# kcroker/Gadget-2.0.7-ngravs

Hardware: AMD Instinct MI355X
Metric: particle-steps/s (tree+PM) (higher is better)
Workload: dtype f64

## Files before the change

### gadget-2.0.7-ngravs_amd/__init__.py

```python
import ctypes as C
import os
import subprocess

import numpy as np

from . import abi, ic
from .abi import (Config, Particles, Stats, make_config, WALK_GROUP, WALK_STRICT,
                  LAW_NONE, LAW_NEWTON, LAW_NEG_NEWTON, LAW_YUKAWA, LAW_COLOYUK, LAW_BAMBAM, LAW_SOURCEBAM, LAW_TARGETBAM)

_HERE = os.path.dirname(os.path.abspath(__file__))
LIB_PATH = os.path.join(_HERE, "libngravs_hip.so")
_LIB = None

EXPORTS = [
    "ngravs_abi_version", "ngravs_build_info", "ngravs_config_default", "ngravs_create", "ngravs_create_with_laws", "ngravs_destroy",
    "ngravs_last_walk_kernel", "ngravs_shortrange_table_with_laws", "ngravs_user_table_eval",
    "ngravs_set_fatal_handler", "ngravs_set_opening", "ngravs_set_walk_mode", "ngravs_set_softening", "ngravs_dd_record_bytes", "ngravs_get_config", "ngravs_set_tuning",
    "ngravs_memcpy", "ngravs_device_alloc", "ngravs_device_free",
    "ngravs_set_particles",
    "ngravs_set_old_acc", "ngravs_update_particles", "ngravs_force_update_tree", "ngravs_domain_decomposition", "ngravs_discard_grav_pm",
    "ngravs_force_treebuild", "ngravs_gravity_tree",
    "ngravs_pmforce_periodic", "ngravs_compute_accelerations", "ngravs_get_accel", "ngravs_get_stats", "ngravs_walk_unopened",
    "ngravs_get_domain", "ngravs_get_keys", "ngravs_get_order", "ngravs_get_shard", "ngravs_last_error",
    "ngravs_peano_hilbert_key", "ngravs_peano_keys", "ngravs_shortrange_table", "ngravs_direct_sum", "ngravs_direct_sum_targets",
    "ngravs_dd_num_local", "ngravs_dd_local_extent", "ngravs_dd_set_extent", "ngravs_get_domain_extent", "ngravs_dd_set_toptree",
    "ngravs_dd_get_toptree", "ngravs_dd_peano_order", "ngravs_dd_leaf_sums", "ngravs_dd_target_bounds", "ngravs_dd_keep_margin", "ngravs_dd_pack", "ngravs_dd_get_dest",
    "ngravs_dd_pack_leaves", "ngravs_dd_set_top", "ngravs_dd_recv_buffer", "ngravs_dd_apply_migration", "ngravs_dd_set_halo",
    "ngravs_dd_leaf_sums_kept", "ngravs_dd_pack_leaves_kept", "ngravs_dd_refresh_halo", "ngravs_dd_update_top", "ngravs_dd_get_kept",
    "ngravs_dd_set_ids", "ngravs_dd_get_ids",
    "ngravs_pm_slab_begin", "ngravs_pm_slab_pack", "ngravs_pm_slab_unpack", "ngravs_pm_slab_bytes",
]
HOST_EXPORTS = ["ngravs_host_comm_selftest", "ngravs_host_kept_step", "ngravs_host_toptree_borrow", "ngravs_host_domain_decomposition", "ngravs_host_domain_owners", "ngravs_host_domain_halo",
                "ngravs_host_plan_free", "ngravs_host_pmforce_periodic", "ngravs_host_compute_accelerations", "ngravs_host_split",
                "ngravs_host_pm_seconds", "ngravs_host_toptree_init", "ngravs_host_toptree_from_children", "ngravs_host_toptree_adapt",
                "ngravs_host_toptree_free", "ngravs_host_import_request", "ngravs_host_import_request_margin"]
RCCL_LIB_PATH = os.path.join(_HERE, "libngravs_rccl.so")
RCCL_EXPORTS = ["ngravs_rccl_selftest", "ngravs_rccl_unique_id", "ngravs_rccl_create", "ngravs_rccl_fill", "ngravs_rccl_destroy", "ngravs_rccl_stats",
                "ngravs_rccl_last_error", "ngravs_rccl_world", "ngravs_rccl_barrier", "ngravs_rccl_set_timeout"]

# ... 43 lines not shown
        L.ngravs_get_keys.argtypes = [C.c_void_p, C.c_void_p, C.c_int]
        L.ngravs_get_order.argtypes = [C.c_void_p, C.c_void_p, C.c_int]
        L.ngravs_get_shard.argtypes = [C.c_void_p, C.c_void_p, C.c_void_p]
        L.ngravs_peano_keys.argtypes = [C.c_void_p, C.c_void_p, C.c_int64, C.c_void_p, C.c_double, C.c_int, C.c_void_p]
        L.ngravs_shortrange_table.argtypes = [C.c_void_p, C.c_void_p, C.c_void_p]
        L.ngravs_direct_sum.argtypes = [C.c_void_p, C.c_void_p, C.c_int64, C.c_void_p]
        L.ngravs_direct_sum_targets.argtypes = [C.c_void_p, C.c_void_p, C.c_void_p, C.c_void_p, C.c_int64, C.c_void_p]
        L.ngravs_dd_local_extent.argtypes = [C.c_void_p, C.c_void_p, C.c_void_p]
        L.ngravs_dd_set_extent.argtypes = [C.c_void_p, C.c_void_p, C.c_void_p]
        L.ngravs_get_config.argtypes = [C.c_void_p, C.c_void_p]
        L.ngravs_host_split.argtypes = [C.c_void_p, C.c_void_p, C.c_int64, C.c_int, C.c_double, C.c_void_p]
        L.ngravs_dd_pack.argtypes = [C.c_void_p, C.c_int, C.c_void_p, C.c_int, C.c_int, C.c_void_p, C.c_void_p, C.c_void_p]
        L.ngravs_host_toptree_init.argtypes = [C.c_void_p, C.c_int]
        L.ngravs_host_toptree_from_children.argtypes = [C.c_void_p, C.c_void_p, C.c_int32]
        L.ngravs_host_toptree_adapt.argtypes = [C.c_void_p, C.c_void_p, C.c_double, C.c_int, C.c_void_p]
        L.ngravs_host_toptree_free.argtypes = [C.c_void_p]
        L.ngravs_host_toptree_free.restype = None
        L.ngravs_host_import_request.argtypes = [C.c_void_p, C.c_void_p, C.c_void_p, C.c_void_p, C.c_void_p, C.c_int, C.c_void_p, C.c_void_p]
        L.ngravs_dd_apply_migration.argtypes = [C.c_void_p, C.c_void_p, C.c_int64]
        L.ngravs_dd_set_halo.argtypes = [C.c_void_p, C.c_void_p, C.c_int64]
        L.ngravs_dd_set_ids.argtypes = [C.c_void_p, C.c_void_p, C.c_int]
        L.ngravs_create_with_laws.argtypes = [C.c_void_p, C.c_void_p, C.c_int, C.c_void_p]
        L.ngravs_last_walk_kernel.argtypes = [C.c_void_p]
        L.ngravs_shortrange_table_with_laws.argtypes = [C.c_void_p, C.c_void_p, C.c_int, C.c_void_p, C.c_void_p]
        L.ngravs_user_table_eval.argtypes = [C.c_void_p, C.c_double, C.c_double, C.c_double, C.c_void_p, C.c_int64, C.c_void_p,
                                             C.c_void_p]
        L.ngravs_dd_get_ids.argtypes = [C.c_void_p, C.c_void_p, C.c_int]
        _LIB = L
    return _LIB


def shard_range(n, rank, world_size):
    lo = (n * rank) // world_size
    hi = (n * (rank + 1)) // world_size
    lo = (lo // 64) * 64
    hi = n if rank + 1 == world_size else (hi // 64) * 64
    return lo, hi - lo


def peano_hilbert_key(x, y, z, bits):
    return int(lib().ngravs_peano_hilbert_key(int(x), int(y), int(z), int(bits)))


def shortrange_table(cfg):
    ng = cfg.n_gravs
    force = np.zeros((ng, ng, abi.NTAB))
# ... 28 lines not shown
    return out, err.value


def _ptr(a):
    return a.ctypes.data if a is not None else None


class Engine:

    def __init__(self, cfg, user_fns=None):
        self.cfg = cfg
        self._h = C.c_void_p()
        self._user_arr, nfns, self._user_keep = abi.user_registry(user_fns)
        rc = lib().ngravs_create_with_laws(C.byref(cfg), self._user_arr, nfns, C.byref(self._h))
        if rc != 0:
            msg = lib().ngravs_last_error(None)
            self.status = rc
            raise NgravsError("ngravs_create failed with status %d (no HIP device or bad wiring): %s" % (rc, msg.decode() if msg else ""))
        self._keep = []
        self.n = 0

    def last_walk_kernel(self):
        return int(lib().ngravs_last_walk_kernel(self._h))

    def close(self):
        if self._h:
            lib().ngravs_destroy(self._h)
            self._h = C.c_void_p()

    def __del__(self):
        try:
            self.close()
        except Exception:
            pass

    def _check(self, rc, what):
        if rc != 0:
            msg = lib().ngravs_last_error(self._h)
            raise NgravsError("%s failed: status %d (%s)" % (what, rc, msg.decode() if msg else ""))

    def _host_columns(self, pos, mass, ptype, old_acc, active, grav_pm, grav_cost=None):
        pos = np.ascontiguousarray(pos, dtype=np.float64)
        mass = np.ascontiguousarray(mass, dtype=np.float64)
        ptype = np.ascontiguousarray(ptype, dtype=np.int32)
        p = Particles()
        p.n = len(pos)
# ... 176 lines not shown
```

### gadget-2.0.7-ngravs_amd/csrc/capi.hip

```cpp
#include "engine.hpp"
#include "../../include/ngravs_peano.h"
#include <chrono>
#include <cmath>

static thread_local std::string g_create_error;

void ngravs_report(ngravs_ctx *ctx, int code, const std::string &msg)
{
  if(ctx)
    ctx->last_error = msg;
  else
    g_create_error = msg;
  if(ctx && ctx->on_fatal)
    ctx->on_fatal(code, msg.c_str());
  else
    fprintf(stderr, "task %d: endrun called with an error level of %d (%s)\n", ctx ? ctx->cfg.rank : 0, code, msg.c_str());
}

__global__ void k_pack_strided_f64(const unsigned char *src, long long stride, int ncomp, long long n, double *dst)
{
  long long i = blockIdx.x * (long long)blockDim.x + threadIdx.x;
  if(i >= n)
    return;
  const double *s = reinterpret_cast<const double *>(src + i * stride);
// ... 234 lines not shown
  std::string why;
  int rc = check_config(cfg, why);
  if(rc == NGRAVS_OK)
    rc = user_check_config(cfg, fns, nfns, why);
  if(rc != NGRAVS_OK)
    {
      ngravs_report(nullptr, rc, why);
      return rc;
    }
  int ndev = 0;
  if(hipGetDeviceCount(&ndev) != hipSuccess || ndev <= 0)
    {
      ngravs_report(nullptr, NGRAVS_ERR_NO_DEVICE, "no HIP device: libngravs_hip has no CPU fallback");
      return NGRAVS_ERR_NO_DEVICE;
    }
  if(cfg->device < 0 || cfg->device >= ndev)
    return NGRAVS_ERR_ARG;
  ngravs_ctx *c = new ngravs_ctx;
  c->cfg = *cfg;
  c->user_fns.assign(fns, fns + nfns);
  memset(&c->stats, 0, sizeof(c->stats));
  if(hipSetDevice(cfg->device) != hipSuccess || hipStreamCreate(&c->stream) != hipSuccess ||
     hipEventCreate(&c->ev0) != hipSuccess || hipEventCreate(&c->ev1) != hipSuccess ||
     hipEventCreate(&c->evk0) != hipSuccess || hipEventCreate(&c->evk1) != hipSuccess)
    {
      delete c;
      return NGRAVS_ERR_NO_DEVICE;
    }
  if(cfg->pmgrid)
    {
      c->asmth = cfg_asmth(cfg);
      c->rcut = cfg_rcut(cfg);
    }
  *out = c;
  return NGRAVS_OK;
}

extern "C" void ngravs_destroy(ngravs_ctx *c)
{
  if(!c)
    return;
  (void)hipSetDevice(c->cfg.device);
  (void)hipStreamSynchronize(c->stream);
  pm_release(c);
  pmslab_release(c);
  c->in_cost.release();
  c->in_pos.release();
// ... 46 lines not shown
  c->lat.release();
  c->walk_stack.release();
  c->walk_counters.release();
  c->walk_ovf.release();
  c->walk_tlist.release();
  c->walk_tmp.release();
  c->lvl_table.release();
  c->r_acc.release();
  c->r_pm.release();
  c->r_oldacc.release();
  c->r_nint.release();
  c->pm_rho.release();
  c->pm_phi.release();
  c->pm_force.release();
  c->pm_orig.release();
  c->out_tmp.release();
  c->out_tmpf.release();
  (void)hipEventDestroy(c->ev0);
  (void)hipEventDestroy(c->ev1);
  (void)hipEventDestroy(c->evk0);
  (void)hipEventDestroy(c->evk1);
  for(hipEvent_t e : c->ev_batch)
    (void)hipEventDestroy(e);
  (void)hipStreamDestroy(c->stream);
  delete c;
}

extern "C" void ngravs_set_fatal_handler(ngravs_ctx *ctx, ngravs_fatal_fn fn)
{
  if(ctx)
    ctx->on_fatal = fn;
}

extern "C" int ngravs_set_opening(ngravs_ctx *c, double theta, double errtol)
{
  if(!c)
    return NGRAVS_ERR_ARG;
  c->cfg.err_tol_theta = theta;
  c->cfg.err_tol_force_acc = errtol;
  return NGRAVS_OK;
}

extern "C" int ngravs_set_softening(ngravs_ctx *c, const double force_softening[NGRAVS_NTYPES])
{
  if(!c || !force_softening)
    return NGRAVS_ERR_ARG;
// ... 49 lines not shown
    }
  else if(k == "walk_root")
    t.walk_root = iv != 0;
  else if(k == "walk_compact")
    t.walk_compact = iv != 0;
  else if(k == "walk_spread" && iv >= 0 && iv <= 64 && (iv & (iv - 1)) == 0)
    t.walk_spread = (int)iv;
  else if(k == "walk_sg" && iv >= 0 && iv <= 16)
    t.walk_sg = (int)iv;
  else if(k == "walk_ring" && iv >= 0 && iv <= 1)
    t.walk_ring = (int)iv;
  else if(k == "walk_ring_k" && iv >= 0 && iv <= 8)
    t.walk_ring_k = (int)iv;
  else if(k == "walk_nleaf" && iv >= -1 && iv <= 8)
    t.walk_nleaf = (int)iv;
  else if(k == "walk_exact_reach")
    t.walk_exact_reach = iv != 0;
  else if(k == "sort_full")
    t.sort_full = iv != 0;
  else if(k == "tree_levelwise")
    t.tree_levelwise = iv != 0;
  else if(k == "dd_keep" && v >= 0 && v <= 0.25)
    t.dd_keep = v;
  else
    {
      ngravs_report(c, NGRAVS_ERR_ARG, "ngravs_set_tuning: unknown name or value out of range: " + k);
      return NGRAVS_ERR_ARG;
    }
  return NGRAVS_OK;
}

extern "C" int ngravs_memcpy(ngravs_ctx *c, void *dst, const void *src, int64_t bytes, int kind)
{
  if(!c || bytes < 0 || kind < 1 || kind > 3 || (bytes > 0 && (!dst || !src)))
    return NGRAVS_ERR_ARG;
  if(bytes == 0)
    return NGRAVS_OK;
  (void)hipSetDevice(c->cfg.device);
  HIP_TRY(c, hipStreamSynchronize(c->stream));
  HIP_TRY(c, hipMemcpy(dst, src, (size_t)bytes, kind == 1 ? hipMemcpyHostToDevice : (kind == 2 ? hipMemcpyDeviceToHost : hipMemcpyDeviceToDevice)));
  return NGRAVS_OK;
}

extern "C" int ngravs_device_alloc(ngravs_ctx *c, void **ptr, int64_t bytes)
{
  if(!c || !ptr || bytes < 0)
// ... 42 lines not shown
}

static double ev_ms(ngravs_ctx *c);

static int set_particles_impl(ngravs_ctx *c, const ngravs_particles_t *p, bool keep_tree)
{
  if(!c || !p || p->n < 0 || (p->n > 0 && (!p->pos || !p->mass || !p->type)))
    return NGRAVS_ERR_ARG;
  if(p->n == 0 && keep_tree)
    {
      if(!c->have_particles || c->n_local != 0)
        return NGRAVS_ERR_STATE;
      c->tree_stale = c->have_tree;
      return NGRAVS_OK;
    }
  if(p->n == 0)
    {
      (void)hipSetDevice(c->cfg.device);
      c->n = c->n_local = 0;
      c->own_order_nlocal = -1;
      c->sort_low = 35;
      c->all_active = true;
      c->walk_ia_ratio = 0;
      c->walk_unit_state = 4;
      c->have_particles = true;
      c->have_order = c->have_tree = c->have_pm = c->have_acc = false;
      c->top.on = false;
      c->pm_parked = false;
      return NGRAVS_OK;
    }
  const bool keep_halo = keep_tree && c->n_local != c->n;
  if(keep_tree && (!c->have_order || !c->have_tree || p->n != c->n_local))
    {
      ngravs_report(c, NGRAVS_ERR_STATE, "ngravs_update_particles: needs a built tree over the same own particles");
      return NGRAVS_ERR_STATE;
    }
  if(p->n >= (1ll << 31) - 64)
    {
      ngravs_report(c, NGRAVS_ERR_ARG, "int particle indices (reference All.MaxPart is int): n must be < 2^31");
      return NGRAVS_ERR_ARG;
    }
  (void)hipSetDevice(c->cfg.device);
  const int64_t n = p->n;
  if(c->in_pos.ensure(3 * n) || c->in_mass.ensure(n) || c->in_oldacc.ensure(n) || c->in_type.ensure(n) || c->in_active.ensure(n) ||
     (!keep_tree && c->in_cost.ensure(n)))
    {
// ... 75 lines not shown
        }
      HIP_TRY(c, hipMemcpyAsync(c->in_type.p, h, sizeof(int) * n, hipMemcpyHostToDevice, c->stream));
      HIP_TRY(c, hipStreamSynchronize(c->stream));
    }
  c->all_active = p->active == nullptr;
  if(p->active)
    {
      if(p->on_device)
        hipLaunchKernelGGL(k_pack_active, GRID1(n), 0, c->stream, (const unsigned char *)p->active,
                           (long long)p->active_stride, (long long)n, c->in_active.p);
      else
        {
          c->host_stage.resize((size_t)n);
          for(int64_t i = 0; i < n; i++)
            c->host_stage[i] = ((const unsigned char *)p->active)[i * p->active_stride] ? 1 : 0;
          HIP_TRY(c, hipMemcpyAsync(c->in_active.p, c->host_stage.data(), (size_t)n, hipMemcpyHostToDevice, c->stream));
          HIP_TRY(c, hipStreamSynchronize(c->stream));
        }
    }
  else
    hipLaunchKernelGGL(k_fill_u8, GRID1(n), 0, c->stream, c->in_active.p, (long long)n, (unsigned char)1);
  HIP_TRY(c, hipGetLastError());
  c->walk_ia_ratio = 0;
  c->walk_unit_state = 4;
  c->have_particles = true;
  if(keep_tree)
    c->tree_stale = true;
  else
    {
      c->have_order = c->have_tree = c->have_pm = c->have_acc = false;
      c->top.on = false;
      c->pm_parked = false;
      if(p->grav_pm && c->cfg.pmgrid)
        {
          if(c->pm_orig.ensure(3 * n))
            return NGRAVS_ERR_NOMEM;
          if((rc = upload_column_f64(c, p->grav_pm, p->grav_pm_stride, 3, n, p->on_device, c->pm_orig.p)))
            return rc;
          c->pm_parked = true;
        }
    }
  return NGRAVS_OK;
}

extern "C" int ngravs_set_particles(ngravs_ctx *c, const ngravs_particles_t *p) { return set_particles_impl(c, p, false); }

// ... 156 lines not shown
}

static int ensure_table(ngravs_ctx *c)
{
  if(!c->cfg.pmgrid || c->table_ready)
    return NGRAVS_OK;
  const int ng = c->cfg.n_gravs;
  std::vector<double> h((size_t)(ng * ng + 1) * NTAB);
  host_shortrange_table(&c->cfg, h.data(), nullptr, c->user_fns.data(), (int)c->user_fns.size());
  {
    WalkParams wp;
    make_walk_params(c, &wp);
    for(int t = 0; t < NTAB; t++)
      h[(size_t)ng * ng * NTAB + t] = exp(-wp.ym * (double)t * wp.inv_asmthfac);
  }
  if(c->table.ensure(h.size()))
    return NGRAVS_ERR_NOMEM;
  HIP_TRY(c, hipMemcpyAsync(c->table.p, h.data(), sizeof(double) * h.size(), hipMemcpyHostToDevice, c->stream));
  HIP_TRY(c, hipStreamSynchronize(c->stream));
  c->table_ready = true;
  return NGRAVS_OK;
}

extern "C" int ngravs_gravity_tree(ngravs_ctx *c)
{
  if(!c || !c->have_order)
    return NGRAVS_ERR_STATE;
  (void)hipSetDevice(c->cfg.device);
  int rc;
  if(!c->have_tree)
    {
      int64_t nn = ngravs_force_treebuild(c);
      if(nn < 0)
        return (int)nn;
    }
  else if(c->tree_stale && (rc = ngravs_force_update_tree(c)))
    return rc;
  if((rc = ensure_table(c)))
    return rc;
  if(c->n_local == 0)
    {
      c->stats.t_treewalk = 0;
      c->stats.walk_kernel_ms = 0;
      c->stats.interactions = 0;
      c->stats.n_active = 0;
      c->have_acc = true;
      return NGRAVS_OK;
    }
  HIP_TRY(c, hipEventRecord(c->ev0, c->stream));
  if((rc = walk_run(c)))
    return rc;
  if((rc = walk_finish(c)))
    return rc;
  HIP_TRY(c, hipEventRecord(c->ev1, c->stream));
  c->stats.t_treewalk = ev_ms(c) * 1e-3;
  float kms = 0;
  (void)hipEventSynchronize(c->evk1);
  (void)hipEventElapsedTime(&kms, c->evk0, c->evk1);
  c->stats.walk_kernel_ms = kms;
  double h[2] = {0, 0};
  HIP_TRY(c, hipMemcpyAsync(h, c->red_tmp.p, 2 * sizeof(double), hipMemcpyDeviceToHost, c->stream));
  HIP_TRY(c, hipStreamSynchronize(c->stream));
  c->stats.interactions = h[0];
  c->stats.n_active = (int64_t)h[1];
  c->have_acc = true;
  if(c->cfg.pmgrid && c->cfg.walk_mode == NGRAVS_WALK_GROUP && h[1] > 0 && c->cfg.box_size > 0)
    {
      const double reach = (c->cfg.group_reach > 0 ? c->cfg.group_reach : NGRAVS_GROUP_REACH) * c->asmth;
      const double ntot = c->top.on && c->top.total_count > 0 ? c->top.total_count : (double)c->n;
      const double L = c->cfg.box_size, expect = 4.18879020478639 * reach * reach * reach * ntot / (L * L * L);
      const bool dense = c->walk_ntargets < 0 || c->walk_dense_tlist;
      if(expect > 0 && dense)
        {
          const double f_sg = c->walk_sg >= 4 ? 1.0 : (c->walk_sg >= 2 ? 1857.0 / 1393.0 : 1857.0 / 1079.0);
          const double f_s = c->walk_spread >= 2 ? 1079.0 / 871.0 : 1.0;
          c->walk_ia_ratio = (h[0] / h[1]) / expect * f_sg * f_s;
        }
    }
  if(c->shard_count > 0 && c->extent_override)
    hipLaunchKernelGGL(k_cost_update, GRID1(c->shard_count), 0, c->stream, c->s_idx.p, c->s_active.p, c->r_nint.p,
                       (long long)c->shard_first, (long long)c->shard_count, c->in_cost.p);
  return NGRAVS_OK;
}

extern "C" int ngravs_pmforce_periodic(ngravs_ctx *c)
{
  if(!c || !c->have_particles)
    return NGRAVS_ERR_STATE;
  (void)hipSetDevice(c->cfg.device);
  int rc;
  if(!c->have_order && (rc = ngravs_domain_decomposition(c)))
    return rc;
  if(!c->have_tree)
    {
      int64_t nn = ngravs_force_treebuild(c);
      if(nn < 0)
        return (int)nn;
    }
  else if(c->tree_stale && (rc = ngravs_force_update_tree(c)))
    return rc;
  HIP_TRY(c, hipEventRecord(c->ev0, c->stream));
  if((rc = pm_run(c)))
    return rc;
  HIP_TRY(c, hipEventRecord(c->ev1, c->stream));
  c->stats.t_pm = ev_ms(c) * 1e-3;
  return NGRAVS_OK;
}

extern "C" int ngravs_compute_accelerations(ngravs_ctx *c, int pm_step)
{
  if(!c || !c->have_particles)
    return NGRAVS_ERR_STATE;
  int rc;
  if((rc = domain_decomposition_impl(c, !(pm_step && c->cfg.pmgrid))))
    return rc;
  if(pm_step && c->cfg.pmgrid && (rc = ngravs_pmforce_periodic(c)))
    return rc;
  return ngravs_gravity_tree(c);
}

static int download_strided(ngravs_ctx *c, const void *dsrc, size_t elem, int ncomp, int64_t n, void *dst, int64_t stride,
                            int on_device)
{
  const size_t row = elem * ncomp;
  if(on_device)
    {
      if((size_t)stride != row)
        {
          ngravs_report(c, NGRAVS_ERR_ARG, "device outputs must be contiguous");
          return NGRAVS_ERR_ARG;
        }
      HIP_TRY(c, hipMemcpyAsync(dst, dsrc, row * n, hipMemcpyDeviceToDevice, c->stream));
      HIP_TRY(c, hipStreamSynchronize(c->stream));
      return NGRAVS_OK;
    }
  if((size_t)stride == row)
    {
      HIP_TRY(c, hipMemcpyAsync(dst, dsrc, row * n, hipMemcpyDeviceToHost, c->stream));
      HIP_TRY(c, hipStreamSynchronize(c->stream));
      return NGRAVS_OK;
    }
// ... 196 lines not shown
}

extern "C" int ngravs_get_order(ngravs_ctx *c, int32_t *order, int on_device)
{
  if(!c || !c->have_order || !order)
    return NGRAVS_ERR_STATE;
  (void)hipSetDevice(c->cfg.device);
  return download_strided(c, c->s_idx.p, sizeof(int), 1, c->n, order, sizeof(int), on_device);
}

extern "C" int ngravs_get_shard(ngravs_ctx *c, int64_t *first, int64_t *count)
{
  if(!c || !c->have_order)
    return NGRAVS_ERR_STATE;
  if(first)
    *first = c->shard_first;
  if(count)
    *count = c->shard_count;
  return NGRAVS_OK;
}

extern "C" const char *ngravs_last_error(ngravs_ctx *c) { return c ? c->last_error.c_str() : g_create_error.c_str(); }
extern "C" int ngravs_last_walk_kernel(ngravs_ctx *c) { return c ? c->last_walk_kernel : NGRAVS_ERR_ARG; }

extern "C" int64_t ngravs_peano_hilbert_key(int x, int y, int z, int bits) { return ngravs_ph_key(x, y, z, bits); }

extern "C" int ngravs_peano_keys(ngravs_ctx *c, const double *pos, int64_t n, const double corner[3], double fac, int bits,
                                 int64_t *keys)
{
  if(!c || !pos || !keys || n <= 0 || bits < 1 || bits > 21)
    return NGRAVS_ERR_ARG;
  (void)hipSetDevice(c->cfg.device);
  DevBuf<double> dpos;
  DevBuf<long long> dkeys;
  if(dpos.ensure(3 * n) || dkeys.ensure(n))
    return NGRAVS_ERR_NOMEM;
  int rc = NGRAVS_OK;
  if(hipMemcpyAsync(dpos.p, pos, sizeof(double) * 3 * n, hipMemcpyHostToDevice, c->stream) != hipSuccess)
    rc = NGRAVS_ERR_NO_DEVICE;
  if(!rc)
    rc = dom_keys_only(c, dpos.p, n, corner, fac, bits, dkeys.p);
  if(!rc && hipMemcpyAsync(keys, dkeys.p, sizeof(long long) * n, hipMemcpyDeviceToHost, c->stream) != hipSuccess)
    rc = NGRAVS_ERR_NO_DEVICE;
  (void)hipStreamSynchronize(c->stream);
  dpos.release();
  dkeys.release();
// ... 339 lines not shown
```

### gadget-2.0.7-ngravs_amd/csrc/engine.hpp

```cpp
#pragma once
#include <hip/hip_runtime.h>
#include <cstdint>
#include <cstdio>
#include <cstdlib>
#include <cstring>
#include <string>
#include <vector>
#include "../../include/ngravs_host.h"

#define NG_MAX NGRAVS_MAX_GRAVS
#define NTAB NGRAVS_NTAB
#define TREE_BITS NGRAVS_TREE_BITS
#define FLAG_BUCKET 64
#define FLAG_PSEUDO 128
#define FLAG_PARTIAL 256
#define MAX_LEVELS (TREE_BITS + 1)

struct ngravs_ctx;

#define HIP_TRY(ctx, expr)                                                                        \
  do                                                                                              \
    {                                                                                             \
      hipError_t e__ = (expr);                                                                    \
      if(e__ != hipSuccess)                                                                       \
// ... 106 lines not shown
  UserTabs ut;
};

struct TreeView
{
  const int *first, *count, *child, *flags;
  const int *npart;
  const double4 *geo, *mom;
  int nnodes;
  const int *ltab;
  int ltab_level;
  double ltab_corner[3], ltab_cl;
};

struct Tuning
{
  int walk_fused = 0, walk_waves = 0, walk_lcap = 0, walk_root = 0, walk_compact = 1, walk_spread = 0, walk_exact_reach = 0, walk_sg = 0, walk_nleaf = -1;
  long long walk_batch = 0;
  int sort_full = 0;
  int tree_levelwise = 0;
  double dd_keep = 0;
  int walk_ring = 1;
  int walk_ring_k = 0;
};

#define TOP_CW(ng) (7 + 4 * (ng))
struct TopTree
{
  double total_count = 0;
  bool on = false;
  double import_reach = 0;
  ngravs_toptree h = {0, 0, 0, 0, nullptr, nullptr, nullptr, nullptr, nullptr};
  DevBuf<int> child, leaf;
  DevBuf<int> gcnt;
  DevBuf<unsigned char> info;
  DevBuf<double> gsum;
  DevBuf<int> leaf_owner;
  DevBuf<unsigned long long> reqmask;
  DevBuf<double> leaf_sums;
  DevBuf<int> own_leaf;
  long long own_leaf_n = -1;
  int kept_rank = -1, kept_world = 0;
  std::vector<int> h_leaf_owner;
  std::vector<unsigned char> h_present;
  std::vector<double> h_node_sums;
  DevBuf<int> kept_row;
// ... 98 lines not shown
  DevBuf<int> r_nint;
  int pm_plan_n = 0;
  void *fft_fwd = nullptr, *fft_inv = nullptr;
  DevBuf<double> pm_rho;
  DevBuf<double> pm_force;
  DevBuf<double> pm_phi;
  DevBuf<double> pm_orig;
  DevBuf<double> out_tmp;
  DevBuf<float> out_tmpf;
  std::vector<unsigned char> host_stage;
  ngravs_stats_t stats;
  hipEvent_t ev0 = nullptr, ev1 = nullptr, evk0 = nullptr, evk1 = nullptr;
  std::vector<hipEvent_t> ev_batch;
  int walk_batches = 0;
  int walk_lcap = 0;
  int walk_scap = 0;
  std::string last_error;
  std::vector<ngravs_user_fn_t> user_fns;
  DevBuf<double> user_tab;
  UserTabs user_ut = {};
  bool user_ready = false;
  double user_soft[NGRAVS_NTYPES] = {0, 0, 0, 0, 0, 0};
  int last_walk_kernel = 0;
  DevBuf<double> user_green;
  long long user_green_nk2 = 0;
};

int dom_find_extent(ngravs_ctx *c);
int dom_keys_and_sort(ngravs_ctx *c);
int dom_keys_only(ngravs_ctx *c, const double *d_pos, int64_t n, const double corner[3], double fac, int bits,
                  long long *d_keys);
int dd_local_extent(ngravs_ctx *c, double lo[3], double hi[3]);
void dd_apply_extent(ngravs_ctx *c, const double lo[3], const double hi[3]);
int dd_set_toptree(ngravs_ctx *c, int nnode, const int *child);
int dd_leaf_sums(ngravs_ctx *c, void **dev_sums, int64_t *count);
int dd_pack(ngravs_ctx *c, int what, const int *leaf_owner, int nranks, int me, int64_t *counts, void **dev_records, int64_t *nrec);
int dd_apply_migration(ngravs_ctx *c, const void *dev_records, int64_t nrec);
int dd_get_dest(ngravs_ctx *c, const int *leaf_owner, int *dest);
int dd_target_bounds(ngravs_ctx *c, double out[2]);
int dd_pack_leaves(ngravs_ctx *c, const unsigned long long *reqmask, int nranks, int me, int64_t *counts, void **dev_records, int64_t *nrec);
int dd_set_top(ngravs_ctx *c, const double *node_sums, const unsigned char *present);
int dd_set_halo(ngravs_ctx *c, const void *dev_records, int64_t nrec);
int dd_leaf_sums_kept(ngravs_ctx *c, void **dev_sums, int64_t *count);
int dd_pack_leaves_kept(ngravs_ctx *c, int64_t *counts, void **dev_records, int64_t *nrec);
int dd_refresh_halo(ngravs_ctx *c, const void *dev_records, int64_t nrec);
int dd_update_top(ngravs_ctx *c, const double *node_sums, const double *leaf_len);
int dd_peano_order_own(ngravs_ctx *c, int force);
int dd_fill_ids(ngravs_ctx *c);
// ... 48 lines not shown
```

### gadget-2.0.7-ngravs_amd/csrc/kernels_pm.hip

```cpp
#include "engine.hpp"
#include "pm_common.hpp"
#include <hipfft/hipfft.h>

__global__ void k_cic_deposit(const double4 *__restrict__ s_pm, const unsigned char *__restrict__ s_type,
                              const unsigned char *__restrict__ s_flag, long long n,
                              double to_slab, int N, int ng, const int *__restrict__ t2g_tab, double *__restrict__ rho)
{
  long long i = blockIdx.x * (long long)blockDim.x + threadIdx.x;
  if(i >= n || (s_flag[i] & 2))
    return;
  double4 p = s_pm[i];
  int g = t2g_tab[s_type[i]];
  const long long NZ = N + 2;
  double *grid = rho + (size_t)g * N * N * NZ;
  double dx, dy, dz;
  int sx = cell_of(p.x, to_slab, N, &dx), sy = cell_of(p.y, to_slab, N, &dy), sz = cell_of(p.z, to_slab, N, &dz);
  int sxx = sx + 1 == N ? 0 : sx + 1, syy = sy + 1 == N ? 0 : sy + 1, szz = sz + 1 == N ? 0 : sz + 1;
  double m = p.w;
  atomicAdd(&grid[((long long)sx * N + sy) * NZ + sz], m * (1.0 - dx) * (1.0 - dy) * (1.0 - dz));
  atomicAdd(&grid[((long long)sx * N + syy) * NZ + sz], m * (1.0 - dx) * dy * (1.0 - dz));
  atomicAdd(&grid[((long long)sx * N + sy) * NZ + szz], m * (1.0 - dx) * (1.0 - dy) * dz);
  atomicAdd(&grid[((long long)sx * N + syy) * NZ + szz], m * (1.0 - dx) * dy * dz);
  atomicAdd(&grid[((long long)sxx * N + sy) * NZ + sz], m * (dx) * (1.0 - dy) * (1.0 - dz));
  atomicAdd(&grid[((long long)sxx * N + syy) * NZ + sz], m * (dx)*dy * (1.0 - dz));
// ... 344 lines not shown
  HIP_TRY(c, hipGetLastError());
  return NGRAVS_OK;
}

int pm_deposit(ngravs_ctx *c)
{
  const int N = c->cfg.pmgrid, ng = c->cfg.n_gravs;
  const long long n = c->n;
  if(N <= 0 || !c->cfg.periodic)
    {
      ngravs_report(c, NGRAVS_ERR_ARG, "pmforce_periodic needs PERIODIC and PMGRID");
      return NGRAVS_ERR_ARG;
    }
  const size_t real_elems = (size_t)N * N * (N + 2);
  if(c->pm_rho.ensure(real_elems * ng) || c->pm_phi.ensure(real_elems * ng) || c->r_pm.ensure(3 * n) || c->d_counters.ensure(16))
    return NGRAVS_ERR_NOMEM;
  if(c->pm_plan_n != N)
    {
      pm_release(c);
      c->fft_fwd = new hipfftHandle;
      c->fft_inv = new hipfftHandle;
      FFT_TRY(c, hipfftPlan3d((hipfftHandle *)c->fft_fwd, N, N, N, HIPFFT_D2Z));
      FFT_TRY(c, hipfftPlan3d((hipfftHandle *)c->fft_inv, N, N, N, HIPFFT_Z2D));
      FFT_TRY(c, hipfftSetStream(*(hipfftHandle *)c->fft_fwd, c->stream));
      FFT_TRY(c, hipfftSetStream(*(hipfftHandle *)c->fft_inv, c->stream));
      c->pm_plan_n = N;
    }
  HIP_TRY(c, hipMemcpyAsync(c->d_counters.p + 8, c->cfg.type_to_grav, sizeof(int) * 6, hipMemcpyHostToDevice, c->stream));
  const double L = c->cfg.box_size, to_slab = N / L;
  HIP_TRY(c, hipMemsetAsync(c->pm_rho.p, 0, sizeof(double) * real_elems * ng, c->stream));
  const int bs = 256;
  unsigned nbp = (unsigned)((n + bs - 1) / bs);
  MeshAddr ma;
  ma.N = N;
  ma.brick = 0;
  for(int j = 0; j < 3; j++)
    {
      ma.lo[j] = 0;
      ma.ext[j] = N;
    }
  int rct = pm_deposit_tiles(c, ma, c->pm_rho.p);
  if(rct == 1)
    hipLaunchKernelGGL(k_cic_deposit, dim3(nbp), dim3(bs), 0, c->stream, c->s_pm.p, c->s_type.p, c->s_active.p, n, to_slab, N, ng,
                       c->d_counters.p + 8, c->pm_rho.p);
  else if(rct)
    return rct;
  HIP_TRY(c, hipGetLastError());
  return NGRAVS_OK;
}

// ... 82 lines not shown
```

### gadget-2.0.7-ngravs_amd/csrc/kernels_walk.hip

```cpp
#include "engine.hpp"
#include "walk_device.hpp"
#include "eval_asm.inc"
#include <hipcub/hipcub.hpp>
#include <type_traits>

__device__ __forceinline__ double bam_eta(int law, double target, double m, double N, double eps)
{
  if(law == NGRAVS_LAW_BAMBAM)
    return 4.0 * M_PI * eps / (target + m / N);
  if(law == NGRAVS_LAW_SOURCEBAM)
    return 4.0 * M_PI * eps * N / m;
  return 4.0 * M_PI * eps / target;
}
__device__ __forceinline__ double bam_accel(int law, double target, double m, double r, double N, double eps)
{
  double eta = bam_eta(law, target, m, N, eps), rho = 2 * target * m / M_PI;
  double reta = r * eta, reta2 = reta * reta, eta3 = eta * eta * eta;
  if(reta < 0.1)
    return rho * eta3 * (2.0 * r / 3.0 - 4.0 * reta2 * r / 5.0 + 6.0 * reta2 * reta2 * r / 7.0);
  return rho * eta3 * (atan(reta) / (reta2 * eta) - 1.0 / (reta * eta * (1 + reta2)));
}
__device__ __forceinline__ double bam_spline(int law, double target, double m, double r, double N, double eps)
{
  double eta = bam_eta(law, target, m, N, eps), rho = 2 * target * m / M_PI;
// ... 2103 lines not shown
  c->walk_dense_tlist = false;
  const bool imports = c->n_local != c->n;
  if((c->all_active && !imports) || c->shard_count <= 0 || !c->tune.walk_compact)
    return NGRAVS_OK;
  const int n = (int)c->shard_count;
  if(c->walk_tlist.ensure((size_t)n) || c->walk_counters.ensure(32))
    return NGRAVS_ERR_NOMEM;
  hipcub::CountingInputIterator<int> idx((int)c->shard_first);
  hipcub::TransformInputIterator<bool, ActiveFlag, const unsigned char *> flags(c->s_active.p + c->shard_first, ActiveFlag());
  size_t bytes = 0;
  HIP_TRY(c, hipcub::DeviceSelect::Flagged(nullptr, bytes, idx, flags, c->walk_tlist.p, c->walk_counters.p + 24, n, c->stream));
  if(c->walk_tmp.ensure(bytes))
    return NGRAVS_ERR_NOMEM;
  HIP_TRY(c, hipcub::DeviceSelect::Flagged(c->walk_tmp.p, bytes, idx, flags, c->walk_tlist.p, c->walk_counters.p + 24, n, c->stream));
  int cnt = 0;
  HIP_TRY(c, hipMemcpyAsync(&cnt, c->walk_counters.p + 24, sizeof(int), hipMemcpyDeviceToHost, c->stream));
  HIP_TRY(c, hipStreamSynchronize(c->stream));
  if(4ll * cnt < 3ll * n || imports)
    c->walk_ntargets = cnt;
  c->walk_dense_tlist = imports && 4ll * cnt >= 3ll * c->n_local;
  return NGRAVS_OK;
}

template <int NG, bool PM, bool YUK, bool TAB_LDS, bool LATT, bool USR = false>
static int launch_group2_t(ngravs_ctx *c, const WalkParams &wp, int *glist = nullptr, int nlist = 0)
{
  const int S0 = c->walk_spread > 1 ? c->walk_spread : 1, G0 = (WAVE / S0) * (glist ? c->walk_sg : 1);
  int S = S0;
  if(glist)
    {
      const int want = nlist <= 4096 ? 64 : (nlist <= 65536 ? 8 : 1);
      S = want > S0 ? want : S0;
    }
  const int G = WAVE / S;
  int ncu = 256;
  hipDeviceProp_t prop;
  if(hipGetDeviceProperties(&prop, c->cfg.device) == hipSuccess && prop.multiProcessorCount > 0)
    ncu = prop.multiProcessorCount;
  const size_t fixed = ((PM && TAB_LDS) ? sizeof(double) * (wp.ntab_lds + wp.exp_tab) * NTAB : 0) + 40 * sizeof(double);
  int waves = (int)((160 * 1024 - fixed) / GW2_WAVE_LDS);
  int per_cu = 1;
  if(waves > GW_MAXWAVES)
    waves = GW_MAXWAVES;
  if(waves < 1)
    waves = 1;
  size_t lds = fixed + (size_t)waves * GW2_WAVE_LDS;
  long long ngroups = glist ? (long long)nlist * (G0 / G) : (walk_tcount(c) + G - 1) / G;
  long long nblk = (long long)ncu * per_cu;
  if(nblk > (ngroups + waves - 1) / waves)
    nblk = (ngroups + waves - 1) / waves;
  if(nblk < 1)
    nblk = 1;
  if(c->walk_stack.ensure((size_t)nblk * waves * (GW_STACK + (size_t)NG * GW2_ITEMS)) || c->walk_counters.ensure(32))
    return NGRAVS_ERR_NOMEM;
  if(glist)
    HIP_TRY(c, hipMemsetAsync(c->walk_counters.p + 8, 0, sizeof(int) * 8, c->stream));
  else
    HIP_TRY(c, hipMemsetAsync(c->walk_counters.p, 0, sizeof(int) * 32, c->stream));
  auto kern = k_walk_group2<NG, PM, YUK, TAB_LDS, LATT, 0, USR>;
  HIP_TRY(c, hipFuncSetAttribute(reinterpret_cast<const void *>(kern), hipFuncAttributeMaxDynamicSharedMemorySize, (int)lds));
  hipLaunchKernelGGL(kern, dim3((unsigned)nblk), dim3(waves * 64), lds, c->stream, tree_view(c), c->s_pm.p,
                     c->s_type.p, c->s_oldacc.p, c->s_active.p, LATT ? c->lat.p : c->table.p, wp, (long long)c->shard_first,
                     walk_tcount(c), c->walk_counters.p, c->walk_stack.p, c->walk_counters.p + 1, c->r_acc.p,
                     c->r_nint.p, (int *)nullptr, (int *)nullptr, 0ll, glist ? (long long)nlist : 0ll, 0, 0, glist, S, G0, walk_tlist(c), 1);
  return NGRAVS_OK;
}

template <int NG, bool PM, bool YUK, bool TAB_LDS, bool LATT, bool USR = false> static int launch_group3_t(ngravs_ctx *c, const WalkParams &wp)
{
  int ncu = 256;
  hipDeviceProp_t prop;
  if(hipGetDeviceProperties(&prop, c->cfg.device) == hipSuccess && prop.multiProcessorCount > 0)
    ncu = prop.multiProcessorCount;
  const size_t fixed = ((PM && TAB_LDS) ? sizeof(double) * (wp.ntab_lds + wp.exp_tab) * NTAB : 0) + 40 * sizeof(double);
  int waves = (int)((160 * 1024 - fixed) / GW2_WAVE_LDS);
  if(waves > GW2_MAXWAVES)
    waves = GW2_MAXWAVES;
  if(c->tune.walk_waves > 0 && c->tune.walk_waves < waves)
    waves = c->tune.walk_waves;
  if(waves < 1)
    waves = 1;
  const size_t lds = fixed + (size_t)waves * GW2_WAVE_LDS;
  const int S = c->walk_spread > 1 ? c->walk_spread : 1, G = WAVE / S;
  const long long ngroups = (walk_tcount(c) + G - 1) / G;
  int SG = (PM && (c->walk_ntargets < 0 || c->walk_dense_tlist)) ? 4 : 1;
  if(SG == 4)
    {
      const double r = c->walk_ia_ratio;
      int st = c->walk_unit_state;
      if(r > 0)
        {
          if(st == 4)
            st = r > 2.0 ? 1 : (r > 1.4 ? 2 : 4);
          else if(st == 2)
            st = r > 2.0 ? 1 : (r < 1.2 ? 4 : 2);
          else
// ... 453 lines not shown
```

### include/ngravs_hip.h

```cpp
#ifndef NGRAVS_HIP_H
#define NGRAVS_HIP_H

#include <stdint.h>
#include <stddef.h>

#ifdef __cplusplus
extern "C" {
#endif

#define NGRAVS_ABI_VERSION 3
#define NGRAVS_MAX_GRAVS 3
#define NGRAVS_NTYPES 6
#define NGRAVS_NTAB 2048
#define NGRAVS_ASMTH 1.25
#define NGRAVS_RCUT 4.5
#define NGRAVS_BITS_PER_DIMENSION 18
#define NGRAVS_GROUP_REACH 4.5
#define NGRAVS_TREE_BITS 21

typedef enum {
  NGRAVS_LAW_NONE = 0,
  NGRAVS_LAW_NEWTON = 1,
  NGRAVS_LAW_NEG_NEWTON = 2,
  NGRAVS_LAW_YUKAWA = 3,
// ... 94 lines not shown
  NGRAVS_USER_SPLINE = 1,
  NGRAVS_USER_GREENS = 2,
  NGRAVS_USER_NORMED = 3
} ngravs_user_kind;
typedef struct {
  int32_t kind;
  int32_t reserved;
  ngravs_gravity_fn fn;
} ngravs_user_fn_t;
typedef enum {
  NGRAVS_KERNEL_NONE = 0,
  NGRAVS_KERNEL_STRICT = 1,
  NGRAVS_KERNEL_STRICT_USER = 2,
  NGRAVS_KERNEL_GROUP = 3,
  NGRAVS_KERNEL_GROUP_USER = 4
} ngravs_walk_kernel_id;

int ngravs_abi_version(void);
const char *ngravs_build_info(void);
void ngravs_config_default(ngravs_config_t *cfg);
int ngravs_create(const ngravs_config_t *cfg, ngravs_ctx **out);
int ngravs_create_with_laws(const ngravs_config_t *cfg, const ngravs_user_fn_t *fns, int nfns, ngravs_ctx **out);
int ngravs_last_walk_kernel(ngravs_ctx *ctx);
void ngravs_destroy(ngravs_ctx *ctx);
void ngravs_set_fatal_handler(ngravs_ctx *ctx, ngravs_fatal_fn fn);
int ngravs_set_opening(ngravs_ctx *ctx, double err_tol_theta, double err_tol_force_acc);
int ngravs_set_walk_mode(ngravs_ctx *ctx, int walk_mode);
int ngravs_set_softening(ngravs_ctx *ctx, const double force_softening[NGRAVS_NTYPES]);
int ngravs_get_config(ngravs_ctx *ctx, ngravs_config_t *out);
int ngravs_set_tuning(ngravs_ctx *ctx, const char *name, double value);
int ngravs_memcpy(ngravs_ctx *ctx, void *dst, const void *src, int64_t bytes, int kind);
int ngravs_device_alloc(ngravs_ctx *ctx, void **ptr, int64_t bytes);
int ngravs_device_free(ngravs_ctx *ctx, void *ptr);

int ngravs_set_particles(ngravs_ctx *ctx, const ngravs_particles_t *p);
int ngravs_update_particles(ngravs_ctx *ctx, const ngravs_particles_t *p);
int ngravs_set_old_acc(ngravs_ctx *ctx, const double *old_acc, int64_t stride, int on_device);

int ngravs_domain_decomposition(ngravs_ctx *ctx);
int ngravs_discard_grav_pm(ngravs_ctx *ctx);
int64_t ngravs_force_treebuild(ngravs_ctx *ctx);
int ngravs_force_update_tree(ngravs_ctx *ctx);
int ngravs_gravity_tree(ngravs_ctx *ctx);
int ngravs_pmforce_periodic(ngravs_ctx *ctx);
int ngravs_compute_accelerations(ngravs_ctx *ctx, int pm_step);

// ... 64 lines not shown
```

Measured before the change: 609.8 million.

## Overlap PM solve with tree walk on CU-masked streams

```diff
diff --git a/gadget-2.0.7-ngravs_amd/__init__.py b/gadget-2.0.7-ngravs_amd/__init__.py
--- a/gadget-2.0.7-ngravs_amd/__init__.py
+++ b/gadget-2.0.7-ngravs_amd/__init__.py
@@ -14,7 +14,7 @@
 
 EXPORTS = [
     "ngravs_abi_version", "ngravs_build_info", "ngravs_config_default", "ngravs_create", "ngravs_create_with_laws", "ngravs_destroy",
-    "ngravs_last_walk_kernel", "ngravs_shortrange_table_with_laws", "ngravs_user_table_eval",
+    "ngravs_last_walk_kernel", "ngravs_last_pm_cus", "ngravs_cu_probe", "ngravs_shortrange_table_with_laws", "ngravs_user_table_eval",
     "ngravs_set_fatal_handler", "ngravs_set_opening", "ngravs_set_walk_mode", "ngravs_set_softening", "ngravs_dd_record_bytes", "ngravs_get_config", "ngravs_set_tuning",
     "ngravs_memcpy", "ngravs_device_alloc", "ngravs_device_free",
     "ngravs_set_particles",
@@ -104,6 +104,8 @@
         L.ngravs_dd_set_ids.argtypes = [C.c_void_p, C.c_void_p, C.c_int]
         L.ngravs_create_with_laws.argtypes = [C.c_void_p, C.c_void_p, C.c_int, C.c_void_p]
         L.ngravs_last_walk_kernel.argtypes = [C.c_void_p]
+        L.ngravs_last_pm_cus.argtypes = [C.c_void_p]
+        L.ngravs_cu_probe.argtypes = [C.c_void_p, C.c_int, C.c_int, C.c_void_p]
         L.ngravs_shortrange_table_with_laws.argtypes = [C.c_void_p, C.c_void_p, C.c_int, C.c_void_p, C.c_void_p]
         L.ngravs_user_table_eval.argtypes = [C.c_void_p, C.c_double, C.c_double, C.c_double, C.c_void_p, C.c_int64, C.c_void_p,
                                              C.c_void_p]
@@ -178,6 +180,14 @@
 
     def last_walk_kernel(self):
         return int(lib().ngravs_last_walk_kernel(self._h))
+
+    def last_pm_cus(self):
+        return int(lib().ngravs_last_pm_cus(self._h))
+
+    def cu_probe(self, which, nblocks=2048):
+        out = np.zeros(nblocks, dtype=np.int32)
+        self._check(lib().ngravs_cu_probe(self._h, which, nblocks, out.ctypes.data), "ngravs_cu_probe")
+        return out
 
     def close(self):
         if self._h:
diff --git a/gadget-2.0.7-ngravs_amd/csrc/capi.hip b/gadget-2.0.7-ngravs_amd/csrc/capi.hip
--- a/gadget-2.0.7-ngravs_amd/csrc/capi.hip
+++ b/gadget-2.0.7-ngravs_amd/csrc/capi.hip
@@ -280,7 +280,8 @@
   memset(&c->stats, 0, sizeof(c->stats));
   if(hipSetDevice(cfg->device) != hipSuccess || hipStreamCreate(&c->stream) != hipSuccess ||
      hipEventCreate(&c->ev0) != hipSuccess || hipEventCreate(&c->ev1) != hipSuccess ||
-     hipEventCreate(&c->evk0) != hipSuccess || hipEventCreate(&c->evk1) != hipSuccess)
+     hipEventCreate(&c->evk0) != hipSuccess || hipEventCreate(&c->evk1) != hipSuccess || hipEventCreate(&c->ev_fork) != hipSuccess ||
+     hipEventCreate(&c->ev_pm0) != hipSuccess || hipEventCreate(&c->ev_pm1) != hipSuccess || hipEventCreate(&c->ev_walk) != hipSuccess)
     {
       delete c;
       return NGRAVS_ERR_NO_DEVICE;
@@ -373,6 +374,18 @@
   (void)hipEventDestroy(c->evk1);
   for(hipEvent_t e : c->ev_batch)
     (void)hipEventDestroy(e);
+  (void)hipEventDestroy(c->ev_fork);
+  (void)hipEventDestroy(c->ev_pm0);
+  (void)hipEventDestroy(c->ev_pm1);
+  (void)hipEventDestroy(c->ev_walk);
+  if(c->pm_stream)
+    {
+      (void)hipStreamSynchronize(c->pm_stream);
+      (void)hipStreamSynchronize(c->walk_stream);
+      (void)hipStreamDestroy(c->pm_stream);
+      (void)hipStreamDestroy(c->walk_stream);
+    }
+  c->probe_out.release();
   (void)hipStreamDestroy(c->stream);
   delete c;
 }
@@ -468,6 +481,8 @@
     t.tree_levelwise = iv != 0;
   else if(k == "dd_keep" && v >= 0 && v <= 0.25)
     t.dd_keep = v;
+  else if(k == "pm_cus" && (iv == -1 || (iv >= 0 && iv <= 32 && iv % 8 == 0)))
+    t.pm_cus = (int)iv;
   else
     {
       ngravs_report(c, NGRAVS_ERR_ARG, "ngravs_set_tuning: unknown name or value out of range: " + k);
@@ -556,6 +571,7 @@
       c->sort_low = 35;
       c->all_active = true;
       c->walk_ia_ratio = 0;
+      c->pm_solo_steps = 0, c->pm_auto_cus = -1;
       c->walk_unit_state = 4;
       c->have_particles = true;
       c->have_order = c->have_tree = c->have_pm = c->have_acc = false;
@@ -677,6 +693,7 @@
     hipLaunchKernelGGL(k_fill_u8, GRID1(n), 0, c->stream, c->in_active.p, (long long)n, (unsigned char)1);
   HIP_TRY(c, hipGetLastError());
   c->walk_ia_ratio = 0;
+  c->pm_solo_steps = 0, c->pm_auto_cus = -1;
   c->walk_unit_state = 4;
   c->have_particles = true;
   if(keep_tree)
@@ -879,7 +896,66 @@
   return NGRAVS_OK;
 }
 
-extern "C" int ngravs_gravity_tree(ngravs_ctx *c)
+static bool pm_cu_bit(int R, int b)
+{
+  const int x = b / 32, k = b - 33 * x;
+  return b < 256 && k >= 0 && k % 8 == 0 && k / 8 < R / 8;
+}
+
+static int masked_streams(ngravs_ctx *c, int R)
+{
+  if(c->pm_stream && c->pm_stream_cus == R)
+    return NGRAVS_OK;
+  if(!c->device_cus)
+    {
+      hipDeviceProp_t prop;
+      HIP_TRY(c, hipGetDeviceProperties(&prop, c->cfg.device));
+      c->device_cus = prop.multiProcessorCount;
+    }
+  if(c->device_cus != 256 || R < 8 || R > 32 || R % 8)
+    return NGRAVS_ERR_ARG;
+  if(c->pm_stream)
+    {
+      HIP_TRY(c, hipStreamSynchronize(c->pm_stream));
+      HIP_TRY(c, hipStreamSynchronize(c->walk_stream));
+      (void)hipStreamDestroy(c->pm_stream);
+      (void)hipStreamDestroy(c->walk_stream);
+      c->pm_stream = c->walk_stream = nullptr;
+      c->pm_stream_cus = 0;
+    }
+  uint32_t mp[8] = {0}, mw[8] = {0};
+  for(int b = 0; b < 256; b++)
+    (pm_cu_bit(R, b) ? mp : mw)[b / 32] |= 1u << (b % 32);
+  hipStream_t sp = nullptr, sw = nullptr;
+  if(hipExtStreamCreateWithCUMask(&sp, 8, mp) != hipSuccess || hipExtStreamCreateWithCUMask(&sw, 8, mw) != hipSuccess)
+    {
+      if(sp)
+        (void)hipStreamDestroy(sp);
+      (void)hipGetLastError();
+      return NGRAVS_ERR_NO_DEVICE;
+    }
+  uint32_t gp[8] = {0}, gw[8] = {0};
+  if(hipExtStreamGetCUMask(sp, 8, gp) != hipSuccess || hipExtStreamGetCUMask(sw, 8, gw) != hipSuccess || memcmp(gp, mp, sizeof mp) ||
+     memcmp(gw, mw, sizeof mw))
+    {
+      (void)hipStreamDestroy(sp);
+      (void)hipStreamDestroy(sw);
+      (void)hipGetLastError();
+      return NGRAVS_ERR_NO_DEVICE;
+    }
+  c->pm_stream = sp;
+  c->walk_stream = sw;
+  c->pm_stream_cus = R;
+  return NGRAVS_OK;
+}
+
+static bool overlap_eligible(const ngravs_ctx *c)
+{
+  return c->cfg.pmgrid && c->cfg.periodic && c->cfg.world_size == 1 && !c->top.on && c->cfg.walk_mode == NGRAVS_WALK_GROUP &&
+         c->n > 0 && c->n_local > 0;
+}
+
+static int gravity_tree_impl(ngravs_ctx *c, hipEvent_t pm_done)
 {
   if(!c || !c->have_order)
     return NGRAVS_ERR_STATE;
@@ -905,8 +981,22 @@
       return NGRAVS_OK;
     }
   HIP_TRY(c, hipEventRecord(c->ev0, c->stream));
-  if((rc = walk_run(c)))
-    return rc;
+  const bool masked = (pm_done || (c->tune.pm_cus > 0 && overlap_eligible(c))) && masked_streams(c, pm_done ? c->pm_stream_cus : c->tune.pm_cus) == NGRAVS_OK;
+  if(masked)
+    {
+      HIP_TRY(c, hipStreamWaitEvent(c->walk_stream, c->ev0, 0));
+      {
+        OnStream on(c, c->walk_stream, c->device_cus - c->pm_stream_cus);
+        if((rc = walk_run(c)))
+          return rc;
+      }
+      HIP_TRY(c, hipEventRecord(c->ev_walk, c->walk_stream));
+      HIP_TRY(c, hipStreamWaitEvent(c->stream, c->ev_walk, 0));
+    }
+  else if((rc = walk_run(c)))
+    return rc;
+  if(pm_done)
+    HIP_TRY(c, hipStreamWaitEvent(c->stream, pm_done, 0));
   if((rc = walk_finish(c)))
     return rc;
   HIP_TRY(c, hipEventRecord(c->ev1, c->stream));
@@ -940,6 +1030,21 @@
   return NGRAVS_OK;
 }
 
+extern "C" int ngravs_gravity_tree(ngravs_ctx *c) { return gravity_tree_impl(c, nullptr); }
+
+static int pm_on_masked_stream(ngravs_ctx *c)
+{
+  HIP_TRY(c, hipEventRecord(c->ev_fork, c->stream));
+  HIP_TRY(c, hipStreamWaitEvent(c->pm_stream, c->ev_fork, 0));
+  OnStream on(c, c->pm_stream, c->pm_stream_cus);
+  HIP_TRY(c, hipEventRecord(c->ev_pm0, c->stream));
+  int rc = pm_run(c);
+  if(rc)
+    return rc;
+  HIP_TRY(c, hipEventRecord(c->ev_pm1, c->stream));
+  return NGRAVS_OK;
+}
+
 extern "C" int ngravs_pmforce_periodic(ngravs_ctx *c)
 {
   if(!c || !c->have_particles)
@@ -956,6 +1061,17 @@
     }
   else if(c->tree_stale && (rc = ngravs_force_update_tree(c)))
     return rc;
+  if(c->tune.pm_cus > 0 && overlap_eligible(c) && masked_streams(c, c->tune.pm_cus) == NGRAVS_OK)
+    {
+      if((rc = pm_on_masked_stream(c)))
+        return rc;
+      float ms = 0;
+      HIP_TRY(c, hipEventSynchronize(c->ev_pm1));
+      (void)hipEventElapsedTime(&ms, c->ev_pm0, c->ev_pm1);
+      HIP_TRY(c, hipStreamWaitEvent(c->stream, c->ev_pm1, 0));
+      c->stats.t_pm = ms * 1e-3;
+      return NGRAVS_OK;
+    }
   HIP_TRY(c, hipEventRecord(c->ev0, c->stream));
   if((rc = pm_run(c)))
     return rc;
@@ -964,6 +1080,32 @@
   return NGRAVS_OK;
 }
 
+static const double PM_CU_SCALE[4] = {17.75, 9.07, 6.16, 4.74};
+static const double PM_FIT_MARGIN = 1.05, PM_SHARE_COST = 1.04;
+static int choose_pm_cus(ngravs_ctx *c)
+{
+  if(!overlap_eligible(c))
+    return 0;
+  if(c->tune.pm_cus >= 0)
+    return c->tune.pm_cus;
+  if(c->pm_auto_cus >= 0)
+    return c->pm_auto_cus;
+  if(c->pm_solo_steps < 2 || c->pm_solo_ms <= 0 || c->walk_solo_ms <= 0)
+    return 0;
+  c->pm_auto_cus = 0;
+  for(int m = 1; m <= 4; m++)
+    {
+      const double walk = c->walk_solo_ms * 256.0 / (256 - 8 * m);
+      if(c->pm_solo_ms * PM_CU_SCALE[m - 1] * PM_FIT_MARGIN < walk)
+        {
+          if(walk * PM_SHARE_COST < 0.99 * (c->pm_solo_ms + c->walk_solo_ms))
+            c->pm_auto_cus = 8 * m;
+          break;
+        }
+    }
+  return c->pm_auto_cus;
+}
+
 extern "C" int ngravs_compute_accelerations(ngravs_ctx *c, int pm_step)
 {
   if(!c || !c->have_particles)
@@ -971,9 +1113,38 @@
   int rc;
   if((rc = domain_decomposition_impl(c, !(pm_step && c->cfg.pmgrid))))
     return rc;
-  if(pm_step && c->cfg.pmgrid && (rc = ngravs_pmforce_periodic(c)))
-    return rc;
-  return ngravs_gravity_tree(c);
+  c->last_pm_cus = 0;
+  if(!(pm_step && c->cfg.pmgrid))
+    return ngravs_gravity_tree(c);
+  const int R = choose_pm_cus(c);
+  if(R > 0 && masked_streams(c, R) == NGRAVS_OK)
+    {
+      int64_t nn = ngravs_force_treebuild(c);
+      if(nn < 0)
+        return (int)nn;
+      if((rc = pm_on_masked_stream(c)))
+        return rc;
+      if((rc = gravity_tree_impl(c, c->ev_pm1)))
+        return rc;
+      float ms = 0;
+      (void)hipEventElapsedTime(&ms, c->ev_pm0, c->ev_pm1);
+      c->stats.t_pm = ms * 1e-3;
+      c->last_pm_cus = R;
+      if(c->tune.pm_cus < 0 && ms > c->stats.walk_kernel_ms)
+        c->pm_auto_cus = R < 32 ? R + 8 : 0;
+      return NGRAVS_OK;
+    }
+  if((rc = ngravs_pmforce_periodic(c)))
+    return rc;
+  if((rc = ngravs_gravity_tree(c)))
+    return rc;
+  if(overlap_eligible(c) && c->tune.pm_cus < 0 && c->pm_auto_cus < 0)
+    {
+      c->pm_solo_ms = c->stats.t_pm * 1e3;
+      c->walk_solo_ms = c->stats.walk_kernel_ms;
+      c->pm_solo_steps++;
+    }
+  return NGRAVS_OK;
 }
 
 static int download_strided(ngravs_ctx *c, const void *dsrc, size_t elem, int ncomp, int64_t n, void *dst, int64_t stride,
@@ -1216,6 +1387,42 @@
 
 extern "C" const char *ngravs_last_error(ngravs_ctx *c) { return c ? c->last_error.c_str() : g_create_error.c_str(); }
 extern "C" int ngravs_last_walk_kernel(ngravs_ctx *c) { return c ? c->last_walk_kernel : NGRAVS_ERR_ARG; }
+extern "C" int ngravs_last_pm_cus(ngravs_ctx *c) { return c ? c->last_pm_cus : NGRAVS_ERR_ARG; }
+
+#define CU_PROBE_LDS (96 * 1024)
+__global__ void k_cu_probe(int *out, int n)
+{
+  extern __shared__ int probe_lds[];
+  if(threadIdx.x != 0)
+    return;
+  unsigned xcc = 0, hw = 0;
+  asm volatile("s_getreg_b32 %0, hwreg(HW_REG_XCC_ID)" : "=s"(xcc));
+  asm volatile("s_getreg_b32 %0, hwreg(HW_REG_HW_ID)" : "=s"(hw));
+  probe_lds[0] = (int)(((xcc & 15u) << 8) | ((hw >> 8) & 0xffu));
+  const unsigned long long t0 = wall_clock64();
+  while(wall_clock64() - t0 < 2000)
+    __builtin_amdgcn_s_sleep(8);
+  if((int)blockIdx.x < n)
+    out[blockIdx.x] = probe_lds[0];
+}
+
+extern "C" int ngravs_cu_probe(ngravs_ctx *c, int which, int nblocks, int32_t *cu_ids)
+{
+  if(!c || !cu_ids || nblocks < 1 || nblocks > 65536 || which < 0 || which > 2)
+    return NGRAVS_ERR_ARG;
+  if(which > 0 && !c->pm_stream)
+    return NGRAVS_ERR_STATE;
+  (void)hipSetDevice(c->cfg.device);
+  hipStream_t s = which == 0 ? c->stream : (which == 1 ? c->pm_stream : c->walk_stream);
+  if(c->probe_out.ensure((size_t)nblocks))
+    return NGRAVS_ERR_NOMEM;
+  HIP_TRY(c, hipFuncSetAttribute(reinterpret_cast<const void *>(k_cu_probe), hipFuncAttributeMaxDynamicSharedMemorySize, CU_PROBE_LDS));
+  hipLaunchKernelGGL(k_cu_probe, dim3((unsigned)nblocks), dim3(64), CU_PROBE_LDS, s, c->probe_out.p, nblocks);
+  HIP_TRY(c, hipGetLastError());
+  HIP_TRY(c, hipMemcpyAsync(cu_ids, c->probe_out.p, sizeof(int) * nblocks, hipMemcpyDeviceToHost, s));
+  HIP_TRY(c, hipStreamSynchronize(s));
+  return NGRAVS_OK;
+}
 
 extern "C" int64_t ngravs_peano_hilbert_key(int x, int y, int z, int bits) { return ngravs_ph_key(x, y, z, bits); }
 
diff --git a/gadget-2.0.7-ngravs_amd/csrc/engine.hpp b/gadget-2.0.7-ngravs_amd/csrc/engine.hpp
--- a/gadget-2.0.7-ngravs_amd/csrc/engine.hpp
+++ b/gadget-2.0.7-ngravs_amd/csrc/engine.hpp
@@ -152,6 +152,7 @@
   double dd_keep = 0;
   int walk_ring = 1;
   int walk_ring_k = 0;
+  int pm_cus = -1;
 };
 
 #define TOP_CW(ng) (7 + 4 * (ng))
@@ -296,8 +297,35 @@
   bool user_ready = false;
   double user_soft[NGRAVS_NTYPES] = {0, 0, 0, 0, 0, 0};
   int last_walk_kernel = 0;
+  hipStream_t pm_stream = nullptr, walk_stream = nullptr;
+  int pm_stream_cus = 0;
+  int device_cus = 0;
+  int stream_cus = 0;
+  int last_pm_cus = 0;
+  double pm_solo_ms = 0, walk_solo_ms = 0;
+  int pm_solo_steps = 0;
+  int pm_auto_cus = -1;
+  hipEvent_t ev_fork = nullptr, ev_pm0 = nullptr, ev_pm1 = nullptr, ev_walk = nullptr;
+  DevBuf<int> probe_out;
   DevBuf<double> user_green;
   long long user_green_nk2 = 0;
+};
+
+struct OnStream
+{
+  ngravs_ctx *c;
+  hipStream_t s0;
+  int n0;
+  OnStream(ngravs_ctx *c_, hipStream_t s, int cus) : c(c_), s0(c_->stream), n0(c_->stream_cus)
+  {
+    c->stream = s;
+    c->stream_cus = cus;
+  }
+  ~OnStream()
+  {
+    c->stream = s0;
+    c->stream_cus = n0;
+  }
 };
 
 int dom_find_extent(ngravs_ctx *c);
diff --git a/gadget-2.0.7-ngravs_amd/csrc/kernels_pm.hip b/gadget-2.0.7-ngravs_amd/csrc/kernels_pm.hip
--- a/gadget-2.0.7-ngravs_amd/csrc/kernels_pm.hip
+++ b/gadget-2.0.7-ngravs_amd/csrc/kernels_pm.hip
@@ -390,10 +390,10 @@
       c->fft_inv = new hipfftHandle;
       FFT_TRY(c, hipfftPlan3d((hipfftHandle *)c->fft_fwd, N, N, N, HIPFFT_D2Z));
       FFT_TRY(c, hipfftPlan3d((hipfftHandle *)c->fft_inv, N, N, N, HIPFFT_Z2D));
-      FFT_TRY(c, hipfftSetStream(*(hipfftHandle *)c->fft_fwd, c->stream));
-      FFT_TRY(c, hipfftSetStream(*(hipfftHandle *)c->fft_inv, c->stream));
       c->pm_plan_n = N;
     }
+  FFT_TRY(c, hipfftSetStream(*(hipfftHandle *)c->fft_fwd, c->stream));
+  FFT_TRY(c, hipfftSetStream(*(hipfftHandle *)c->fft_inv, c->stream));
   HIP_TRY(c, hipMemcpyAsync(c->d_counters.p + 8, c->cfg.type_to_grav, sizeof(int) * 6, hipMemcpyHostToDevice, c->stream));
   const double L = c->cfg.box_size, to_slab = N / L;
   HIP_TRY(c, hipMemsetAsync(c->pm_rho.p, 0, sizeof(double) * real_elems * ng, c->stream));
diff --git a/gadget-2.0.7-ngravs_amd/csrc/kernels_walk.hip b/gadget-2.0.7-ngravs_amd/csrc/kernels_walk.hip
--- a/gadget-2.0.7-ngravs_amd/csrc/kernels_walk.hip
+++ b/gadget-2.0.7-ngravs_amd/csrc/kernels_walk.hip
@@ -2149,6 +2149,16 @@
   return NGRAVS_OK;
 }
 
+static int walk_cus(const ngravs_ctx *c)
+{
+  if(c->stream_cus > 0)
+    return c->stream_cus;
+  hipDeviceProp_t prop;
+  if(hipGetDeviceProperties(&prop, c->cfg.device) == hipSuccess && prop.multiProcessorCount > 0)
+    return prop.multiProcessorCount;
+  return 256;
+}
+
 template <int NG, bool PM, bool YUK, bool TAB_LDS, bool LATT, bool USR = false>
 static int launch_group2_t(ngravs_ctx *c, const WalkParams &wp, int *glist = nullptr, int nlist = 0)
 {
@@ -2160,10 +2170,7 @@
       S = want > S0 ? want : S0;
     }
   const int G = WAVE / S;
-  int ncu = 256;
-  hipDeviceProp_t prop;
-  if(hipGetDeviceProperties(&prop, c->cfg.device) == hipSuccess && prop.multiProcessorCount > 0)
-    ncu = prop.multiProcessorCount;
+  const int ncu = walk_cus(c);
   const size_t fixed = ((PM && TAB_LDS) ? sizeof(double) * (wp.ntab_lds + wp.exp_tab) * NTAB : 0) + 40 * sizeof(double);
   int waves = (int)((160 * 1024 - fixed) / GW2_WAVE_LDS);
   int per_cu = 1;
@@ -2195,10 +2202,7 @@
 
 template <int NG, bool PM, bool YUK, bool TAB_LDS, bool LATT, bool USR = false> static int launch_group3_t(ngravs_ctx *c, const WalkParams &wp)
 {
-  int ncu = 256;
-  hipDeviceProp_t prop;
-  if(hipGetDeviceProperties(&prop, c->cfg.device) == hipSuccess && prop.multiProcessorCount > 0)
-    ncu = prop.multiProcessorCount;
+  const int ncu = walk_cus(c);
   const size_t fixed = ((PM && TAB_LDS) ? sizeof(double) * (wp.ntab_lds + wp.exp_tab) * NTAB : 0) + 40 * sizeof(double);
   int waves = (int)((160 * 1024 - fixed) / GW2_WAVE_LDS);
   if(waves > GW2_MAXWAVES)
diff --git a/include/ngravs_hip.h b/include/ngravs_hip.h
--- a/include/ngravs_hip.h
+++ b/include/ngravs_hip.h
@@ -140,6 +140,8 @@
 int ngravs_create(const ngravs_config_t *cfg, ngravs_ctx **out);
 int ngravs_create_with_laws(const ngravs_config_t *cfg, const ngravs_user_fn_t *fns, int nfns, ngravs_ctx **out);
 int ngravs_last_walk_kernel(ngravs_ctx *ctx);
+int ngravs_last_pm_cus(ngravs_ctx *ctx);
+int ngravs_cu_probe(ngravs_ctx *ctx, int which, int nblocks, int32_t *cu_ids);
 void ngravs_destroy(ngravs_ctx *ctx);
 void ngravs_set_fatal_handler(ngravs_ctx *ctx, ngravs_fatal_fn fn);
 int ngravs_set_opening(ngravs_ctx *ctx, double err_tol_theta, double err_tol_force_acc);
```

Result: faster. 630.0 million (median of 6 runs) (+3.3%).
